# pema99/rust-path-tracer

Hardware: AMD Instinct MI355X
Metric: Mrays/s (higher is better)
Workload: dtype f32

## Files before the change

rust-path-tracer_amd/csrc/k_common.h:

```cpp
#ifndef RPT_K_COMMON_H
#define RPT_K_COMMON_H

#include <hip/hip_runtime.h>
#include <stdint.h>

#include "../../include/rpt/shared_structs.h"
#include "rpt_math.h"

#define RPT_WAVE 64
#define RPT_BLOCK 256
#define RPT_MAX_SAMPLES_IN_FLIGHT 256u

struct F3 { float x, y, z; };
RPT_HD F3 f3(float x, float y, float z) { return F3{x, y, z}; }
RPT_HD F3 f3s(float s) { return F3{s, s, s}; }
RPT_HD F3 operator+(F3 a, F3 b) { return F3{a.x + b.x, a.y + b.y, a.z + b.z}; }
RPT_HD F3 operator-(F3 a, F3 b) { return F3{a.x - b.x, a.y - b.y, a.z - b.z}; }
RPT_HD F3 operator*(F3 a, F3 b) { return F3{a.x * b.x, a.y * b.y, a.z * b.z}; }
RPT_HD F3 operator*(F3 a, float s) { return F3{a.x * s, a.y * s, a.z * s}; }
RPT_HD F3 operator*(float s, F3 a) { return F3{s * a.x, s * a.y, s * a.z}; }
RPT_HD F3 operator/(F3 a, float s) { return F3{a.x / s, a.y / s, a.z / s}; }
RPT_HD F3 operator-(F3 a) { return F3{-a.x, -a.y, -a.z}; }
RPT_HD float dot3(F3 a, F3 b) { return (a.x * b.x) + (a.y * b.y) + (a.z * b.z); }
__device__ __forceinline__ F3 cross3(F3 a, F3 b) {
// ... 69 lines not shown
    uint32_t n_slots;
    uint32_t n_pixels;
    uint32_t group_shift;
    uint32_t q_shift;
};
RPT_HD size_t rpt_pixel_index(uint32_t pxy, uint32_t width) { return (size_t)(pxy >> 16) * width + (pxy & 0xffffu); }

#define FLAG_BOUNCE(f) ((f) & 0xffu)
#define FLAG_LOBE_SPEC(f) (((f) >> 8) & 1u)
#define FLAG_DIM(f) (((f) >> 16) & 0x3fu)
#define MAKE_FLAGS(bounce, spec, dim) (((bounce) & 0xffu) | ((uint32_t)(spec) << 8) | ((uint32_t)(dim) << 16))
#define HIT_MISS 0xffffffffu
#define HIT_PENDING 0xfffffffeu
#define HIT_PARKED 0xfffffffdu
#define HIT_DONE 0xfffffffcu
#define HIT_IDLE 0xfffffffbu

#define Q_LINE 32
enum {  Q_ALIVE0 = 2 * Q_LINE, Q_ALIVE1 = 3 * Q_LINE, Q_REGEN0 = 4 * Q_LINE,
       Q_REGEN1 = 5 * Q_LINE, Q_DRAINED = 6 * Q_LINE, Q_POOL0 = 7 * Q_LINE, Q_POOL1 = 8 * Q_LINE, Q_SPOOL = 9 * Q_LINE, Q_COUNT = 12 * Q_LINE };
#define RPT_Q_SHARDS 16
#define RPT_Q_SHARD_STRIDE 1088
#define RPT_Q_SLACK (RPT_Q_SHARDS * (2048u + 256u))
__host__ __device__ __forceinline__ uint32_t q_position(uint32_t shard, uint32_t e) { return ((((e >> 8) * RPT_Q_SHARDS) | shard) << 8) | (e & 255u); }
__device__ __forceinline__ bool q_filled(const uint32_t *cnt, uint32_t p) {
    return ((((p >> 8) / RPT_Q_SHARDS) << 8) | (p & 255u)) < cnt[((p >> 8) % RPT_Q_SHARDS) * RPT_Q_SHARD_STRIDE];
}
__device__ __forceinline__ void q_extent(const uint32_t *cnt, uint32_t &positions, uint32_t &total) {
    uint32_t most = 0u, sum = 0u;
    for (uint32_t s = 0; s < RPT_Q_SHARDS; ++s) {
        const uint32_t c = cnt[s * RPT_Q_SHARD_STRIDE];
// ... 11 lines not shown
#define RPT_STAT_SHARDS 64
#define RPT_STAT_STRIDE 16

struct DevQueues {
    uint32_t *sky;
    float4 *sh_o;
    float4 *sh_d;
    float4 *sh_c;
    uint32_t *count;
    uint32_t *sky_cnt, *shadow_cnt;
    uint32_t sky_threshold;
    uint32_t known_length;
    uint32_t sky_at_end;
    uint32_t sky_wide_limit;
    uint32_t sky_shard_shift;
    unsigned long long *ray_shards;
    unsigned long long *host_ring;
    uint32_t ring_mask;
};

struct DevStats {
    unsigned long long extension_rays, shadow_rays, sky_evals, light_index_clamped, samples;
    unsigned long long undrained;
};

struct DevConfig {
    rpt_tracing_config c;
    float euler[9];
    float sky_rot[9];
    uint32_t nee_mode;
// ... 73 lines not shown
```

rust-path-tracer_amd/csrc/k_complete.h:

```cpp
#ifndef RPT_K_COMPLETE_H
#define RPT_K_COMPLETE_H

#include "k_path.h"
#include "k_moments.h"

#define RPT_COMPLETE_ROWS 32u
#define RPT_COMPLETE_PITCH 65u
__host__ __device__ __forceinline__ uint32_t complete_rows(uint32_t S) { return S < RPT_COMPLETE_ROWS ? S : RPT_COMPLETE_ROWS; }
__host__ __device__ __forceinline__ size_t complete_lds_bytes(uint32_t S, uint32_t q_shift) {
    return q_shift == 0u ? 0u : (size_t)complete_rows(S) * RPT_COMPLETE_PITCH * sizeof(float4) + (size_t)S * sizeof(unsigned long long);
}
template <uint32_t G>
__device__ __forceinline__ void complete_status_rows(const DevState &st, uint32_t base, uint32_t j0, uint32_t lane, unsigned long long *row_done, uint32_t my_group,
                                                     uint32_t my_shift, unsigned long long q_mask, uint32_t &n_done, uint32_t &n_busy, uint32_t &top) {
    const uint32_t gs = st.group_shift, qs = st.q_shift;
    uint32_t w[G];
#pragma unroll
    for (uint32_t i = 0u; i < G; ++i) w[i] = __float_as_uint(st.hit[base + ((j0 + i) << 6) + lane].y);
#pragma unroll
    for (uint32_t i = 0u; i < G; ++i) {
        const uint32_t row = j0 + i;
        const bool done = w[i] == HIT_DONE;
        const unsigned long long md = rpt_ballot(done), mb = rpt_ballot(!done && w[i] != HIT_IDLE);
        if (qs != 0u && lane == 0u) row_done[row] = md;
        if ((row >> (gs - qs)) == my_group) {
            const uint32_t bits = (uint32_t)((md >> my_shift) & q_mask);
            n_done += (uint32_t)__popc(bits);
            n_busy += (uint32_t)__popc((uint32_t)((mb >> my_shift) & q_mask));
            if (bits != 0u) top = ((row & ((1u << (gs - qs)) - 1u)) << qs) + 32u - (uint32_t)__clz((int)bits);
        }
    }
}
__device__ __forceinline__ uint32_t complete_block_slot(const DevState &st, uint32_t base, uint32_t kb, uint32_t t, uint32_t rows, uint32_t rows_log, uint32_t lane) {
    const uint32_t gs = st.group_shift, qs = st.q_shift;
    const uint32_t g = t >> (rows_log - qs), jl = (kb >> qs) + (t & ((rows >> qs) - 1u));
    return base + (((g << (gs - qs)) | jl) << 6) + lane;
}
template <uint32_t G>
__device__ __forceinline__ bool complete_stage_rows(const DevState &st, uint32_t base, uint32_t kb, uint32_t t0, uint32_t rows, uint32_t rows_log, uint32_t lane, float4 *tile,
                                                    const unsigned long long *row_done, unsigned long long ok_mask) {
    float rx[G], ry[G], rz[G], rw[G];
    uint32_t slot_of[G];
    bool restart = false;
#pragma unroll
    for (uint32_t i = 0u; i < G; ++i) {
        slot_of[i] = complete_block_slot(st, base, kb, t0 + i, rows, rows_log, lane);
        const float4 r = st.rad[slot_of[i]];
        rx[i] = r.x; ry[i] = r.y; rz[i] = r.z; rw[i] = r.w;
    }
#pragma unroll
    for (uint32_t i = 0u; i < G; ++i) {
        const uint32_t slot = slot_of[i], p = slot_pix(st, slot) & 63u, k = slot_k(st, slot);
        tile[(k - kb) * RPT_COMPLETE_PITCH + p] = make_float4(rx[i], ry[i], rz[i], rw[i]);
        const bool mine = ((row_done[(slot - base) >> 6] >> lane) & 1ull) != 0ull && ((ok_mask >> p) & 1ull) != 0ull;
        const uint32_t todo = __float_as_uint(rw[i]);
        if (mine && todo == 0u) st.hit[slot] = make_float2(0.0f, __uint_as_float(HIT_IDLE));
        restart = restart || rpt_ballot(mine && todo != 0u) != 0ull;
    }
    return restart;
}
__device__ __forceinline__ bool complete_restart_rows(const DevState &st, const DevConfig &cfg, uint32_t base, uint32_t kb, uint32_t rows, uint32_t rows_log, uint32_t lane,
                                                      const float4 *tile, const unsigned long long *row_done, unsigned long long ok_mask, uint32_t new_n, uint32_t rng_offset) {
// ... 31 lines not shown
```

rust-path-tracer_amd/csrc/k_complete_body.h:

```cpp
template <uint32_t G>
__device__ __forceinline__ bool RPT_COMPLETE_DIRECT_ROWS(const DevState &st, uint32_t base, uint32_t k0, uint32_t lane, bool ok, uint32_t n_done, float4 &acc RPT_MOM(, float4 &mom)) {
    float rx[G], ry[G], rz[G], rw[G];
    bool restart = false;
#pragma unroll
    for (uint32_t i = 0u; i < G; ++i) {
        const float4 r = st.rad[base + ((k0 + i) << 6) + lane];
        rx[i] = r.x; ry[i] = r.y; rz[i] = r.z; rw[i] = r.w;
    }
#pragma unroll
    for (uint32_t i = 0u; i < G; ++i) {
        const bool mine = ok && k0 + i < n_done;
        if (mine) { acc.x += rx[i]; acc.y += ry[i]; acc.z += rz[i]; acc.w += 1.0f; }
        RPT_MOM(if (mine) mo_add(mom, rx[i], ry[i], rz[i]);)
        const uint32_t todo = __float_as_uint(rw[i]);
        if (mine && todo == 0u) st.hit[base + ((k0 + i) << 6) + lane] = make_float2(0.0f, __uint_as_float(HIT_IDLE));
        restart = restart || rpt_ballot(mine && todo != 0u) != 0ull;
    }
    return restart;
}
__global__ __launch_bounds__(RPT_WAVE) void RPT_COMPLETE_KERNEL(DevState st, DevQueues q, DevConfig cfg, uint32_t iteration, uint32_t final_pass,
                                                                DevStats *stats RPT_MOM(, float4 *moments )) {
    if (!final_pass && q.count[Q_DRAINED] != 0u) return;
    extern __shared__ float4 complete_lds[];
    const uint32_t gs = st.group_shift, qs = st.q_shift, S = 1u << gs, rows = complete_rows(S);
    float4 *tile = complete_lds;
    unsigned long long *row_done = reinterpret_cast<unsigned long long *>(complete_lds + rows * RPT_COMPLETE_PITCH);
    const uint32_t lane = threadIdx.x, base = blockIdx.x << (6u + gs), pix = (blockIdx.x << 6) | lane;
    const bool in_image = pix < st.n_pixels;
    const uint32_t my_group = lane >> (6u - qs), my_shift = (lane & ((64u >> qs) - 1u)) << qs;
    const unsigned long long q_mask = (1ull << (1u << qs)) - 1ull;
    uint32_t n_done = 0u, n_busy = 0u, top = 0u;
    bool nothing_to_do = false;
    if (S >= 8u) {
        for (uint32_t j0 = 0u; j0 < S && !nothing_to_do; j0 += 8u) {
            complete_status_rows<8>(st, base, j0, lane, row_done, my_group, my_shift, q_mask, n_done, n_busy, top);
            nothing_to_do = !final_pass && rpt_ballot(in_image && n_busy == 0u) == 0ull;
        }
    } else if (S == 4u) complete_status_rows<4>(st, base, 0u, lane, row_done, my_group, my_shift, q_mask, n_done, n_busy, top);
    else complete_status_rows<2>(st, base, 0u, lane, row_done, my_group, my_shift, q_mask, n_done, n_busy, top);
    if (nothing_to_do) return;
    const bool ok = in_image && n_busy == 0u && n_done != 0u && top == n_done;
    if (final_pass && in_image && (n_busy != 0u || top != n_done)) {
        atomicAdd(&stats->undrained, (unsigned long long)(n_done + n_busy));
    }
    const unsigned long long ok_mask = rpt_ballot(ok);
    bool started = false;
    if (ok_mask != 0ull) {
        float4 acc = make_float4(0.0f, 0.0f, 0.0f, 0.0f);
        RPT_MOM(float4 mom = make_float4(0.0f, 0.0f, 0.0f, 0.0f);)
        uint2 rs = make_uint2(0u, 0u);
        if (ok) { acc = st.accum[pix]; rs = st.rng[pix]; }
        RPT_MOM(if (ok) mom = moments[pix];)
        const uint32_t new_n = rs.x + n_done;
        uint32_t most = ok ? n_done : 0u;
        for (uint32_t o = 32u; o != 0u; o >>= 1) { const uint32_t other = (uint32_t)__shfl_xor((int)most, (int)o, RPT_WAVE); most = other > most ? other : most; }
        const uint32_t rows_log = 31u - (uint32_t)__clz((int)rows);
        __syncthreads();
        if (qs == 0u) {
            const uint32_t G = S >= 8u ? 8u : S;
            for (uint32_t k0 = 0u; k0 < most; k0 += G) {
                bool restart;
                if (G == 8u) restart = RPT_COMPLETE_DIRECT_ROWS<8>(st, base, k0, lane, ok, n_done, acc RPT_MOM(, mom));
                else if (G == 4u) restart = RPT_COMPLETE_DIRECT_ROWS<4>(st, base, k0, lane, ok, n_done, acc RPT_MOM(, mom));
                else restart = RPT_COMPLETE_DIRECT_ROWS<2>(st, base, k0, lane, ok, n_done, acc RPT_MOM(, mom));
                if (restart) {
#pragma unroll 1
                    for (uint32_t k = k0; k < k0 + G; ++k) {
                        const uint32_t slot = base + (k << 6) + lane, todo = __float_as_uint(st.rad[slot].w);
                        if (ok && k < n_done && todo != 0u) {
                            start_path(st, cfg, slot, new_n + k, rs.y, todo - 1u);
                            started = true;
                        }
                    }
                }
            }
        } else
        for (uint32_t kb = 0u; kb < most; kb += rows) {
            bool restart = false;
            if (rows >= 8u) {
                for (uint32_t t0 = 0u; t0 < rows; t0 += 8u) restart |= complete_stage_rows<8>(st, base, kb, t0, rows, rows_log, lane, tile, row_done, ok_mask);
            } else if (rows == 4u) restart = complete_stage_rows<4>(st, base, kb, 0u, rows, rows_log, lane, tile, row_done, ok_mask);
            else restart = complete_stage_rows<2>(st, base, kb, 0u, rows, rows_log, lane, tile, row_done, ok_mask);
            __syncthreads();
            const uint32_t here = most - kb < rows ? most - kb : rows;
            for (uint32_t kl = 0u; kl < here; ++kl) {
                const float4 r = tile[kl * RPT_COMPLETE_PITCH + lane];
                if (ok && kb + kl < n_done) { acc.x += r.x; acc.y += r.y; acc.z += r.z; acc.w += 1.0f; }
                RPT_MOM(if (ok && kb + kl < n_done) mo_add(mom, r.x, r.y, r.z);)
            }
            if (restart) started |= complete_restart_rows(st, cfg, base, kb, rows, rows_log, lane, tile, row_done, ok_mask, new_n, rs.y);
            __syncthreads();
        }
        if (ok) {
            st.accum[pix] = acc;
            rs.x = new_n;
            st.rng[pix] = rs;
            RPT_MOM(moments[pix] = mom;)
// ... 6 lines not shown
```

rust-path-tracer_amd/csrc/k_path.h:

```cpp
#ifndef RPT_K_PATH_H
#define RPT_K_PATH_H

#include "k_common.h"

__device__ __forceinline__ F3 mat3_mul(const float *m, F3 v) {
    F3 r = f3(m[0], m[1], m[2]) * v.x;
    r = r + (f3(m[3], m[4], m[5]) * v.y);
    r = r + (f3(m[6], m[7], m[8]) * v.z);
    return r;
}

__device__ __forceinline__ void camera_ray(const DevConfig &cfg, uint32_t px, uint32_t py, uint32_t key, F3 &ro, F3 &rd) {
    Rng rng{key, 0u};
    float j1 = rng.next(), j2 = rng.next();
    float sx = (float)px + j1, sy = (float)py + j2;
    float ux = (sx / (float)cfg.c.width) * 2.0f - 1.0f;
    float uy = (1.0f - sy / (float)cfg.c.height) * 2.0f - 1.0f;
    uy *= (float)cfg.c.height / (float)cfg.c.width;
    ro = f3(cfg.c.cam_position[0], cfg.c.cam_position[1], cfg.c.cam_position[2]);
    rd = mat3_mul(cfg.euler, norm3(f3(ux, uy, 1.0f)));
}

__device__ __forceinline__ void start_path(const DevState &st, const DevConfig &cfg, uint32_t slot, uint32_t n, uint32_t offset,
                                           uint32_t todo_after) {
// ... 39 lines not shown
__device__ __forceinline__ void finish_in_side_stage(const DevState &st, const DevConfig &cfg, uint32_t slot, F3 radiance, uint32_t todo) {
    if (st.group_shift == 0u) {
        float4 acc = st.accum[slot];
        acc.x += radiance.x; acc.y += radiance.y; acc.z += radiance.z; acc.w += 1.0f;
        st.accum[slot] = acc;
        uint2 rs = st.rng[slot];
        rs.x += 1u;
        st.rng[slot] = rs;
        if (todo == 0u) st.hit[slot] = make_float2(0.0f, __uint_as_float(HIT_IDLE));
        else start_path(st, cfg, slot, rs.x, rs.y, todo - 1u);
    } else {
        st.rad[slot] = make_float4(radiance.x, radiance.y, radiance.z, __uint_as_float(todo));
        st.hit[slot] = make_float2(0.0f, __uint_as_float(HIT_DONE));
    }
}

#endif
```

rust-path-tracer_amd/csrc/k_shade.h:

```cpp
#ifndef RPT_K_SHADE_H
#define RPT_K_SHADE_H

#include "k_common.h"
#include "k_path.h"

#define RPT_PI_F 3.14159265358979323846f
#define RPT_EPS 0.001f

__device__ __forceinline__ uint32_t image_wrap(int32_t c, uint32_t extent, bool pow2) {
    if (pow2) return (uint32_t)c & (extent - 1u);
    const uint32_t u = (uint32_t)c;
    if (u < extent) return u;
    if (u == extent) return 0u;
    return (uint32_t)((uint64_t)(int64_t)c % (uint64_t)extent);
}
__device__ __forceinline__ float4 lerp4(float4 a, float4 b, float s) {
    return make_float4(a.x + ((b.x - a.x) * s), a.y + ((b.y - a.y) * s), a.z + ((b.z - a.z) * s), a.w + ((b.w - a.w) * s));
}
__device__ __forceinline__ float4 texel_of_u8(uint32_t t) {
    return make_float4(rptm::unorm8((float)(t & 0xffu)), rptm::unorm8((float)((t >> 8) & 0xffu)), rptm::unorm8((float)((t >> 16) & 0xffu)), 1.0f);
}
__device__ __forceinline__ void u8_row_pair(const uint32_t *texels, uint32_t row , uint32_t x0, uint32_t x1, uint32_t width, uint32_t &t0, uint32_t &t1) {
    const bool edge = x0 + 1u >= width;
    uint2 pair;
// ... 107 lines not shown
        m.metallic = make_float4(b.w, 0, 0, 0);
        m.normals = make_float4(0, 0, 0, 0);
        m.has = make_uint4(0u, 0u, 0u, 0u);
    }
    return m;
}


template <int NEE, bool TEXTURED, bool COMPACT>
__device__ __forceinline__ void shade_slot(const DevScene &sc, const DevState &st, const DevQueues &q, const DevConfig &cfg, DevStats *stats,
                                           uint32_t slot, float2 hw, bool active, bool &to_sky, bool &emit_shadow, float4 &sh_o, float4 &sh_d,
                                           float4 &sh_c, bool first ,
                                           uint32_t n_samples, bool &elided ,
                                           bool last_iteration ) {
    const uint32_t hit_tri = __float_as_uint(hw.y);
    if (NEE == RPT_NEE_NONE && last_iteration && active && hit_tri != HIT_MISS) {
        const uint32_t tri_index = hit_tri & 0x7fffffffu;
        const uint32_t m = __float_as_uint(sc.tri_shade[4u * tri_index + 2u].w);
        const float4 e4 = TEXTURED ? sc.materials[6u * m] : sc.mat_lite[2u * m];
        const bool emits = (e4.x != 0.0f || e4.y != 0.0f || e4.z != 0.0f) && (hit_tri >> 31) == 0u;
        if (emits || st.group_shift == 0u) {
            const float4 r4 = st.rad[slot];
            F3 radiance = f3(r4.x, r4.y, r4.z);
            if (emits) {
                const float4 tf = st.thr[slot];
                radiance = radiance + mask_nan3(f3(tf.x, tf.y, tf.z) * f3(e4.x, e4.y, e4.z));
            }
            finish_in_side_stage(st, cfg, slot, radiance, __float_as_uint(r4.w));
        } else {
            st.hit[slot] = make_float2(0.0f, __uint_as_float(HIT_DONE));
        }
        return;
    }
    if (active) {
        const float4 ra = st.ray_a[slot];
        const float2 rb = st.ray_b[slot];
        const F3 ro = f3(ra.x, ra.y, ra.z), rd = f3(ra.w, rb.x, rb.y);
        const float hit_t = hw.x;
        if (hit_tri == HIT_MISS) {
            to_sky = true;
            st.hit[slot] = make_float2(0.0f, __uint_as_float(HIT_PARKED));
            if (first) {
                st.thr[slot] = make_float4(1.0f, 1.0f, 1.0f, __uint_as_float(RPT_FRESH_FLAGS));
                st.rad[slot] = make_float4(0.0f, 0.0f, 0.0f, __uint_as_float(first_path_todo(st, slot, n_samples)));
            }
        } else {
            const float4 tf = first ? make_float4(1.0f, 1.0f, 1.0f, __uint_as_float(RPT_FRESH_FLAGS)) : st.thr[slot];
            F3 throughput = f3(tf.x, tf.y, tf.z);
            F3 radiance = f3s(0.0f);
            uint32_t todo = 0u;
            bool rad_loaded = false;
            auto load_rad = [&]() {
                if (!rad_loaded) {
                    if (first) {
                        todo = first_path_todo(st, slot, n_samples);
                    } else {
                        const float4 r4 = st.rad[slot];
                        radiance = f3(r4.x, r4.y, r4.z);
                        todo = __float_as_uint(r4.w);
                    }
                    rad_loaded = true;
                }
            };
            const uint32_t flags = __float_as_uint(tf.w);
            const uint32_t bounce = FLAG_BOUNCE(flags);
            const bool last_spec = FLAG_LOBE_SPEC(flags) != 0u;
            constexpr bool nee = NEE != RPT_NEE_NONE;
            const bool backface = (hit_tri >> 31) != 0u;
            const uint32_t tri_index = hit_tri & 0x7fffffffu;
            const float4 *ts = sc.tri_shade + 4u * tri_index;
            const float4 s0 = ts[0], s1 = ts[1], s2 = ts[2];
            const Mat mat = load_material<TEXTURED>(sc, __float_as_uint(s2.w));
            const F3 hit = ro + rd * hit_t;

            bool done = false;
            const F3 emissive = xyz4(mat.emissive);
            if (emissive.x != 0.0f || emissive.y != 0.0f || emissive.z != 0.0f) {
                if (backface) {
                    done = true;
                } else if (!nee || bounce == 0u || last_spec) {
                    load_rad();
                    radiance = radiance + mask_nan3(throughput * emissive);
                    done = true;
                } else if (NEE == RPT_NEE_MIS) {
                    const float4 ma = st.mis_a[slot], mb = st.mis_b[slot];
                    const uint32_t code = __float_as_uint(ma.x);
                    F3 contribution = f3s(0.0f);
                    if (code != 0xffffffffu) {
                        const rpt_light_pick_entry e = sc.light_pick[code >> 1];
                        const bool side_b = (code & 1u) != 0u;
                        const uint32_t light_tri = side_b ? e.triangle_index_b : e.triangle_index_a;
                        if (tri_index == light_tri) {
                            const float4 *lr = sc.light_rec + 8u * (code >> 1) + (side_b ? 4u : 0u);
                            const float light_area = side_b ? e.triangle_area_b : e.triangle_area_a;
                            const float light_pick_pdf = side_b ? e.triangle_pick_pdf_b : e.triangle_pick_pdf_a;
                            F3 light_normal = f3(lr[0].w, lr[1].w, lr[2].w);
                            float cos_theta = dot3(light_normal, -rd);
// ... 191 lines not shown
                    throughput = throughput * (spectrum / pdf);
                    new_d = sdir;
                    new_o = hit + sdir * RPT_EPS;
                    if (bounce > cfg.c.min_bounces) {
                        float prob = rptm::fmaxr(throughput.x, rptm::fmaxr(throughput.y, throughput.z));
                        if (rng.next() > prob) {
                            done = true;
                        } else {
                            throughput = throughput * (1.0f / prob);
                        }
                    }
                    new_flags = MAKE_FLAGS(bounce + 1u, spec ? 1u : 0u, rng.dim);
                }
            }

            if (done && !emit_shadow) {
                load_rad();
                finish_in_side_stage(st, cfg, slot, radiance, todo);
            } else {
                if (first) {
                    load_rad();
                    st.rad[slot] = make_float4(radiance.x, radiance.y, radiance.z, __uint_as_float(todo));
                }
                if (!done) {
                    st.thr[slot] = make_float4(throughput.x, throughput.y, throughput.z, __uint_as_float(new_flags));
                    st.ray_a[slot] = make_float4(new_o.x, new_o.y, new_o.z, new_d.x);
                    st.ray_b[slot] = make_float2(new_d.y, new_d.z);
                    st.hit[slot] = make_float2(0.0f, __uint_as_float(HIT_PENDING));
                    sh_d.w = __uint_as_float(slot);
                } else {
                    st.hit[slot] = make_float2(0.0f, __uint_as_float(HIT_PARKED));
                    sh_d.w = __uint_as_float(slot | 0x80000000u);
                }
            }
        }
// ... 136 lines not shown
```

rust-path-tracer_amd/csrc/k_sky_generate.h:

```cpp
#ifndef RPT_K_SKY_GENERATE_H
#define RPT_K_SKY_GENERATE_H

#include "k_shade.h"

#define SKY_EARTH_RADIUS 6360e3f
#define SKY_ATMOSPHERE_RADIUS 6380e3f
#define SKY_H_RAY 8e3f
#define SKY_H_MIE 12e2f

__device__ __forceinline__ float sky_escape(F3 p, F3 d, float r) {
    F3 v = p - f3(0.0f, -SKY_EARTH_RADIUS, 0.0f);
    float b = dot3(v, d);
    float det = b * b - dot3(v, v) + r * r;
    if (det < 0.0f) return -1.0f;
    det = rptm::sqrtr(det);
    float t1 = -b - det;
    float t2 = -b + det;
    return t1 >= 0.0f ? t1 : t2;
}
__device__ __forceinline__ float2 sky_densities(F3 p) {
    float h = rptm::fmaxr(len3(p - f3(0.0f, -SKY_EARTH_RADIUS, 0.0f)) - SKY_EARTH_RADIUS, 0.0f);
    return make_float2(rptm::exp_sky(rptm::div_const_nontiny(-h, SKY_H_RAY, 1.0f / SKY_H_RAY)),
                       rptm::exp_sky(rptm::div_const_nontiny(-h, SKY_H_MIE, 1.0f / SKY_H_MIE)));
}
// ... 75 lines not shown
    uint32_t i = blockIdx.x * RPT_BLOCK + threadIdx.x;
    uint32_t positions, n;
    q_extent(q.sky_cnt, positions, n);
    const uint32_t alive = q.count[Q_ALIVE0 + (iteration & 1u) * Q_LINE];
    const uint32_t drained = q.count[Q_DRAINED];
    if (i == 0u) {
        uint32_t busy = drained ? 0u : (alive | q.count[Q_REGEN0 + (iteration & 1u) * Q_LINE] | (n != 0u ? 1u : 0u));
        if (busy == 0u && drained == 0u) q.count[Q_DRAINED] = 1u;
        __hip_atomic_store(&q.host_ring[iteration & q.ring_mask], ((unsigned long long)(iteration + 1u) << 32) | busy,
                           __ATOMIC_RELEASE, __HIP_MEMORY_SCOPE_SYSTEM);
    }
    if (drained != 0u) return;
    if (q.sky_at_end == 0u && n < q.sky_threshold && alive != 0u) return;
    if (i == 0u && n) atomicAdd(&stats->sky_evals, (unsigned long long)n);
    const uint32_t stride = STRIDED ? gridDim.x * RPT_BLOCK : 0u;
    if (cfg.c.has_skybox == 0u && positions <= q.sky_wide_limit) {
        for (uint32_t m = i >> 4; m < positions; m += stride >> 4) {
            if (!q_filled(q.sky_cnt, m)) {
                if (!STRIDED) break;
                continue;
            }
            const uint32_t slot = q.sky[m];
            const uint32_t lane = __lane_id(), g0 = lane & ~15u, j = lane & 15u;
            float4 ra = st.ray_a[slot];
            float2 rb = st.ray_b[slot];
            F3 ro = f3(ra.x, ra.y, ra.z), rd = f3(ra.w, rb.x, rb.y);
            F3 sky = sky_scatter_wide(cfg.c.sun_direction, ro, rd, j, g0);
            if (j == 0u) {
                const float4 tf = st.thr[slot], r4 = st.rad[slot];
                F3 throughput = f3(tf.x, tf.y, tf.z), radiance = f3(r4.x, r4.y, r4.z);
                radiance = radiance + throughput * sky;
                finish_in_side_stage(st, cfg, slot, radiance, __float_as_uint(r4.w));
            }
            if (!STRIDED) break;
        }
        return;
    }
    for (; i < positions; i += stride) {
        if (!q_filled(q.sky_cnt, i)) {
            if (!STRIDED) break;
            continue;
        }
        uint32_t slot = q.sky[i];
        float4 ra = st.ray_a[slot];
        float2 rb = st.ray_b[slot];
        F3 ro = f3(ra.x, ra.y, ra.z), rd = f3(ra.w, rb.x, rb.y);
        const float4 tf = st.thr[slot], r4 = st.rad[slot];
        F3 throughput = f3(tf.x, tf.y, tf.z), radiance = f3(r4.x, r4.y, r4.z);
        if (cfg.c.has_skybox == 0u) {
            radiance = radiance + throughput * sky_scatter(cfg.c.sun_direction, ro, rd);
        } else {
            F3 rotated = mat3_mul(cfg.sky_rot, rd);
            float u = 0.5f + rptm::atan2r(rotated.z, rotated.x) / (2.0f * RPT_PI_F);
            float v = 1.0f - (0.5f + rptm::asinr(rotated.y) / RPT_PI_F);
            float intensity = cfg.c.sun_direction[3] * (1.0f / 15.0f);
            float4 s = sample_by_lod<false>(sc.skybox, u, v);
            radiance = radiance + throughput * f3(s.x, s.y, s.z) * intensity;
        }
        finish_in_side_stage(st, cfg, slot, radiance, __float_as_uint(r4.w));
        if (!STRIDED) break;
    }
}
// ... 43 lines not shown
```

rust-path-tracer_amd/csrc/k_traverse.h:

```cpp
#ifndef RPT_K_TRAVERSE_H
#define RPT_K_TRAVERSE_H

#include "k_common.h"
#include "k_path.h"
#include "rpt_fastdiv.h"

template <bool SMALL> struct StackElem { typedef uint32_t type; };
template <> struct StackElem<true> { typedef uint16_t type; };
template <typename T> __device__ __forceinline__ void stack_put(T *s, int sp, uint32_t v) { s[sp * RPT_WAVE] = (T)v; }
template <typename T> __device__ __forceinline__ uint32_t stack_get(T *s, int sp) { return (uint32_t)s[sp * RPT_WAVE]; }
struct Stack24 {
    uint16_t *lo;
    uint8_t *hi;
};
__device__ __forceinline__ void stack_put(Stack24 s, int sp, uint32_t v) {
    s.lo[sp * RPT_WAVE] = (uint16_t)v;
    s.hi[sp * RPT_WAVE] = (uint8_t)(v >> 16);
}
__device__ __forceinline__ uint32_t stack_get(Stack24 s, int sp) { return (uint32_t)s.lo[sp * RPT_WAVE] | ((uint32_t)s.hi[sp * RPT_WAVE] << 16); }
template <int K> struct StackBits {
    uint16_t *lo;
    uint32_t hi[K];
};
template <int K> __device__ __forceinline__ void stack_put(StackBits<K> &s, int sp, uint32_t v) {
// ... 672 lines not shown
        __syncthreads();
    }
    const SceneViewLds view = FIRST ? SceneViewLds{lds_scene, sc.lds_pairs, sc.n_triangles, sc.lds_root} : stage_scene_lds<THREADS>(sc, lds_scene);
    const float4 *img_lane = view.img;
    uint32_t stop_first = 0u;
    float order_bias = 0.0f;
    uint16_t *stack = &lds_stack[wave][0][lane];
    F3 ro = f3(0, 0, 0), rd = f3(1, 1, 1), ird = f3(1, 1, 1);
    LdsWalk w;
    lds_walk_begin(view, w);
    w.cur = LDS_DESC_DEAD;
    uint32_t slot = 0u;
    bool have = false;
    bool pool_open = true;
    uint32_t traced = 0u;
    const bool done_here = LAST && st.group_shift != 0u;
    auto last_finish = [&](uint32_t s, const HitRecord &r, uint32_t stopped) -> bool {
        if (!done_here) {
            st.hit[s] = make_float2(r.t, __uint_as_float(r.tri));
            return false;
        }
        if (r.tri == HIT_MISS) return true;
        if (stopped == 0u) {
            const uint32_t m = __float_as_uint(sc.tri_shade[4u * (r.tri & 0x7fffffffu) + 2u].w);
            const float4 e4 = sc.textured != 0u ? sc.materials[6u * m] : sc.mat_lite[2u * m];
            if ((e4.x != 0.0f || e4.y != 0.0f || e4.z != 0.0f) && (r.tri >> 31) == 0u) {
                float4 r4 = st.rad[s];
                const float4 tf = st.thr[s];
                const F3 radiance = f3(r4.x, r4.y, r4.z) + mask_nan3(f3(tf.x, tf.y, tf.z) * f3(e4.x, e4.y, e4.z));
                r4.x = radiance.x; r4.y = radiance.y; r4.z = radiance.z;
                st.rad[s] = r4;
            }
        }
        st.hit[s] = make_float2(0.0f, __uint_as_float(HIT_DONE));
        return false;
    };
    auto last_park = [&](bool park, uint32_t s) {
        const uint32_t shard = (s >> q.sky_shard_shift) % RPT_Q_SHARDS;
        unsigned long long todo_m = rpt_ballot(park);
        while (todo_m != 0ull) {
            const uint32_t leader = (uint32_t)__ffsll((long long)todo_m) - 1u;
            const uint32_t sh = (uint32_t)__builtin_amdgcn_readlane((int)shard, (int)leader);
            const bool mine = park && shard == sh;
            const unsigned long long same = rpt_ballot(mine);
            uint32_t e = 0u;
            if (lane == leader) e = atomicAdd(&q.sky_cnt[sh * RPT_Q_SHARD_STRIDE], (uint32_t)__popcll(same));
            e = (uint32_t)__builtin_amdgcn_readlane((int)e, (int)leader);
            if (mine) {
                e += __builtin_amdgcn_mbcnt_hi((uint32_t)(same >> 32), __builtin_amdgcn_mbcnt_lo((uint32_t)same, 0u));
// ... 231 lines not shown
```

rust-path-tracer_amd/csrc/rpt_hip.hip:

```cpp
#include <algorithm>
#include <cstdlib>
#include <cstring>

#include "rpt_ctx.h"

#include "k_shade.h"
#include "k_complete.h"
#include "k_sky_generate.h"
#include "k_image_order.h"

rpt_knobs rpt_read_knobs() {
    rpt_knobs k;
    auto num = [](const char *name, int lo, int hi, int otherwise) { const char *e = getenv(name); if (!e || !e[0]) return otherwise; const int v = atoi(e); return v < lo ? lo : (v > hi ? hi : v); };
    auto word = [](const char *name) { const char *e = getenv(name); return std::string(e ? e : ""); };
    k.stage_timing = num("RPT_STAGE_TIMING", 0, 2, 0);
    k.upload_timing = num("RPT_UPLOAD_TIMING", 0, 1, 0) == 1;
    k.slot_q_shift = num("RPT_SLOT_Q_SHIFT", 0, 5, -1);
    const std::string so = word("RPT_SHADOW_ORDER"), lo = word("RPT_LAST_ORDER");
    k.shadow_order = so == "near" ? 0 : (so == "fixed" ? 1 : -1);
    k.last_order = lo == "off" ? 4 : (lo == "near" ? 0 : (lo == "opaque" ? 1 : (lo == "small" ? 2 : (lo == "ratio" ? 3 : -1))));
    k.shade_compact = num("RPT_SHADE_COMPACT", 0, 1, -1);
    k.sky_strided = num("RPT_SKY_STRIDED", 0, 1 << 20, -1);
    k.stack_bits = num("RPT_STACK_BITS", 16, 32, 16);
    k.coop_leaves = num("RPT_COOP_LEAVES", 0, 1, -1);
// ... 75 lines not shown
    HIP_TRY(c, hipMemsetAsync(c->ray_shards.p, 0, RPT_STAT_SHARDS * RPT_STAT_STRIDE * sizeof(unsigned long long), c->stream));
    HIP_TRY(c, c->q_count.alloc(Q_WORDS));
    HIP_TRY(c, c->pixel_xy.alloc(np));
    if (np) HIP_TRY(c, hipMemcpy(c->pixel_xy.p, c->pixel_xy_host.data(), np * sizeof(uint32_t), hipMemcpyHostToDevice));
    HIP_TRY(c, hipMemsetAsync(c->q_count.p, 0, Q_WORDS * sizeof(uint32_t), c->stream));
    DevState &s = c->state;
    s = DevState{};
    s.rng = c->rng.p; s.accum = c->accum.p; s.pixel_xy = c->pixel_xy.p; s.n_slots = c->n_slots;
    s.n_pixels = (uint32_t)np; s.group_shift = c->group_shift; s.q_shift = 0;
    DevQueues &q = c->queues;
    q = DevQueues{};
    q.ray_shards = c->ray_shards.p; q.count = c->q_count.p;
    q.sky_cnt = c->q_count.p + Q_COUNT; q.shadow_cnt = q.sky_cnt + RPT_Q_SHARDS * RPT_Q_SHARD_STRIDE;
    q.host_ring = c->host_ring_dev; q.ring_mask = RING - 1;
    q.sky_wide_limit = (uint32_t)std::min<size_t>(c->n_slots / 16, c->sky_wide_cfg);
    q.sky_threshold = 1u; q.sky_at_end = 0u; q.known_length = 0u;
    c->has_state = true;
    return RPT_OK;
}

static uint32_t padded_pixels(uint32_t n_pixels) { return (n_pixels + 63u) & ~63u; }

static void launch_complete(rpt_ctx *c, uint32_t iteration, uint32_t final_pass) {
    if (c->moments_on) {
        k_complete_moments<<<padded_pixels(c->n_pixels) / RPT_WAVE, RPT_WAVE, complete_lds_bytes(1u << c->group_shift, c->state.q_shift), c->stream>>>(c->state, c->queues, c->cfg, iteration,
                                                                                                                                 final_pass, c->dev_stats.p, c->moments.p);
        return;
    }
    k_complete<<<padded_pixels(c->n_pixels) / RPT_WAVE, RPT_WAVE, complete_lds_bytes(1u << c->group_shift, c->state.q_shift), c->stream>>>(c->state, c->queues, c->cfg, iteration, final_pass,
                                                                                                                     c->dev_stats.p);
}
// ... 358 lines not shown
    const uint64_t known_iterations =
        (n_samples <= (1u << c->group_shift) && c->queues.sky_threshold <= 1u) ? (uint64_t)c->cfg.c.max_bounces : 0u;
    HIP_TRY(c, hipSetDevice(c->device));
    const auto t0 = std::chrono::steady_clock::now();
    hipStream_t s = c->stream;
    StageTimer &t = c->timing;
    const uint32_t blocks = rpt_blocks(c->n_slots);
    const bool async = allow_async && known_iterations != 0;
    if (!async && c->async_pending) {
        RPT_TRY(rpt_wait(c));
    }
    if (!async) for (int k = 0; k < RING; ++k) __atomic_store_n(&c->host_ring.p[k], 0ull, __ATOMIC_RELAXED);
    c->call_samples = n_samples;
    c->queues.sky_at_end = known_iterations != 0 ? 1u : 0u;
    c->queues.known_length = known_iterations != 0 ? 1u : 0u;
    c->queues.sky_shard_shift = c->shade_compact ? 11u : 8u;
    static_assert(RPT_BLOCK == 1 << 8 && RPT_BLOCK * RPT_SHADE_ROUNDS == 1 << 11, "sky_shard_shift: slots per workgroup of k_shade");
    t.mark(s, StageTimer::NONE, StageTimer::AT_1);
    c->first_walk_starts = rpt_first_walk_starts_paths(c);
    k_generate_first<<<c->first_walk_starts ? 1u : blocks, RPT_BLOCK, 0, s>>>(c->state, c->queues, c->cfg, n_samples, c->dev_stats.p, c->first_walk_starts ? 1u : 0u);
    c->stats.kernel_launches[RPT_STAGE_GENERATE] += 1;
    t.mark(s, RPT_STAGE_GENERATE, StageTimer::AT_1);

    const uint64_t planned = known_iterations - (async && known_iterations > 1 && c->test_short_batch ? 1u : 0u);
    const bool complete_each = known_iterations == 0 && c->group_shift != 0;
    const uint64_t lag = c->n_slots >= (512u << 10) ? 2 : (c->n_slots >= (128u << 10) ? 3 : LAG);
    const uint64_t it_limit = (uint64_t)n_samples * (uint64_t)(c->cfg.c.max_bounces + 2u) * 16u + 4096u;
    uint64_t it = 0, shade_launches = 0;
    bool drained = c->cfg.c.max_bounces == 0u;
    while (!drained) {
// ... 126 lines not shown
```

rust-path-tracer_amd/csrc/rpt_traverse.hip:

```cpp
#include <hip/hip_runtime.h>

#include <type_traits>

#include "rpt_ctx.h"
#include "k_traverse.h"

namespace {

constexpr int GLOBAL_THREADS = 64;
constexpr int LDS_THREADS = 1024;


template <int STACK>
static int gstream_stack_width(const rpt_ctx *c) {
    if (STACK == 16) return 16;
    const int bits = c->knobs.stack_bits;
    const int w = (c->scene.n_nodes < 65536u && bits <= 16) ? 16 : (c->scene.n_nodes < (1u << 21) && bits <= 21) ? 21 : (c->scene.n_nodes < (1u << 24) && bits <= 24) ? 24 : 32;
    return STACK == 24 && w > 24 ? 24 : w;
}
template <int STACK, typename F>
static void with_stack_width(int width, F &&launch) {
    if constexpr (STACK == 16) launch(std::integral_constant<int, 16>{});
    else if (width == 16) launch(std::integral_constant<int, 16>{});
    else if (width == 21) launch(std::integral_constant<int, 21>{});
// ... 26 lines not shown
}

template <int STACK>
bool launch_nearest(rpt_ctx *c, uint32_t iteration, bool last_without_nee = false ,
                    bool camera_rays = false ,
                    bool start_paths = false ) {
    hipStream_t s = c->stream;
    DevStats *stats = c->dev_stats.p;
    if (STACK == 16 && c->scene.lds_scene) {
        const size_t lds_bytes = (size_t)c->scene.lds_vecs * sizeof(float4);
        uint32_t grid;
        const uint32_t span = lds_stream_span(c, grid);
        const float *cam = c->cfg.c.cam_position;
        if (last_without_nee && c->scene.last_emit_n <= RPT_LAST_EMIT_MAX) {
            k_traverse_nearest_stream<16, LDS_THREADS, RPT_NEAREST_LAST><<<grid, LDS_THREADS, lds_bytes + (size_t)c->scene.last_flip_vecs * sizeof(float4), s>>>(c->scene, c->state, c->queues, iteration, span, 0.0f, 0.0f, 0.0f, c->cfg, 0u, stats);
            return c->state.group_shift != 0u;
        }
        if (camera_rays)
            k_traverse_nearest_stream<16, LDS_THREADS, RPT_NEAREST_FIRST><<<grid, LDS_THREADS, lds_bytes, s>>>(c->scene, c->state, c->queues, iteration, span, cam[0], cam[1], cam[2], c->cfg, start_paths ? c->call_samples : 0u, stats);
        else k_traverse_nearest_stream<16, LDS_THREADS><<<grid, LDS_THREADS, lds_bytes, s>>>(c->scene, c->state, c->queues, iteration, span, 0.0f, 0.0f, 0.0f, c->cfg, 0u, stats);
    } else if (c->scene.gpairs) {
        if (c->fat_leaves) launch_nearest_gstream<STACK, true>(c, iteration);
        else launch_nearest_gstream<STACK, false>(c, iteration);
    } else {
        const uint32_t nb = (c->n_slots + GLOBAL_THREADS - 1) / GLOBAL_THREADS;
        k_traverse_nearest<32, GLOBAL_THREADS><<<nb, GLOBAL_THREADS, 0, s>>>(c->scene, c->state, c->queues, iteration);
    }
    return false;
}

template <int STACK, bool COOP>
// ... 82 lines not shown
```

Baseline: 12860.

## Skip radiance buffer traffic for no-NEE known-length paths via implicit zero state

```diff
diff --git a/rust-path-tracer_amd/csrc/k_common.h b/rust-path-tracer_amd/csrc/k_common.h
--- a/rust-path-tracer_amd/csrc/k_common.h
+++ b/rust-path-tracer_amd/csrc/k_common.h
@@ -107,7 +107,8 @@
 #define HIT_PENDING 0xfffffffeu
 #define HIT_PARKED 0xfffffffdu
 #define HIT_DONE 0xfffffffcu
-#define HIT_IDLE 0xfffffffbu
+#define HIT_DONE_ZERO 0xfffffffbu
+#define HIT_IDLE 0xfffffffau
 
 #define Q_LINE 32
 enum {  Q_ALIVE0 = 2 * Q_LINE, Q_ALIVE1 = 3 * Q_LINE, Q_REGEN0 = 4 * Q_LINE,
@@ -149,6 +150,7 @@
     uint32_t sky_at_end;
     uint32_t sky_wide_limit;
     uint32_t sky_shard_shift;
+    uint32_t implicit_zero;
     unsigned long long *ray_shards;
     unsigned long long *host_ring;
     uint32_t ring_mask;
diff --git a/rust-path-tracer_amd/csrc/k_complete.h b/rust-path-tracer_amd/csrc/k_complete.h
--- a/rust-path-tracer_amd/csrc/k_complete.h
+++ b/rust-path-tracer_amd/csrc/k_complete.h
@@ -8,21 +8,22 @@
 #define RPT_COMPLETE_PITCH 65u
 __host__ __device__ __forceinline__ uint32_t complete_rows(uint32_t S) { return S < RPT_COMPLETE_ROWS ? S : RPT_COMPLETE_ROWS; }
 __host__ __device__ __forceinline__ size_t complete_lds_bytes(uint32_t S, uint32_t q_shift) {
-    return q_shift == 0u ? 0u : (size_t)complete_rows(S) * RPT_COMPLETE_PITCH * sizeof(float4) + (size_t)S * sizeof(unsigned long long);
+    return (size_t)((S + 7u) / 8u) * RPT_WAVE + (q_shift == 0u ? 0u : (size_t)complete_rows(S) * RPT_COMPLETE_PITCH * sizeof(float4) + (size_t)S * sizeof(unsigned long long));
 }
 template <uint32_t G>
-__device__ __forceinline__ void complete_status_rows(const DevState &st, uint32_t base, uint32_t j0, uint32_t lane, unsigned long long *row_done, uint32_t my_group,
-                                                     uint32_t my_shift, unsigned long long q_mask, uint32_t &n_done, uint32_t &n_busy, uint32_t &top) {
+__device__ __forceinline__ void complete_status_rows(const DevState &st, uint32_t base, uint32_t j0, uint32_t lane, unsigned long long *row_done, uint8_t *own_rad, uint32_t my_group, uint32_t my_shift, unsigned long long q_mask, uint32_t &n_done, uint32_t &n_busy, uint32_t &top) {
     const uint32_t gs = st.group_shift, qs = st.q_shift;
     uint32_t w[G];
 #pragma unroll
     for (uint32_t i = 0u; i < G; ++i) w[i] = __float_as_uint(st.hit[base + ((j0 + i) << 6) + lane].y);
+    uint32_t own = 0u;
 #pragma unroll
     for (uint32_t i = 0u; i < G; ++i) {
         const uint32_t row = j0 + i;
-        const bool done = w[i] == HIT_DONE;
+        const bool has_rad = w[i] == HIT_DONE, done = has_rad || w[i] == HIT_DONE_ZERO;
         const unsigned long long md = rpt_ballot(done), mb = rpt_ballot(!done && w[i] != HIT_IDLE);
         if (qs != 0u && lane == 0u) row_done[row] = md;
+        own |= (has_rad ? 1u : 0u) << i;
         if ((row >> (gs - qs)) == my_group) {
             const uint32_t bits = (uint32_t)((md >> my_shift) & q_mask);
             n_done += (uint32_t)__popc(bits);
@@ -30,22 +31,33 @@
             if (bits != 0u) top = ((row & ((1u << (gs - qs)) - 1u)) << qs) + 32u - (uint32_t)__clz((int)bits);
         }
     }
+    own_rad[(j0 >> 3) * RPT_WAVE + lane] = (uint8_t)own;
 }
 __device__ __forceinline__ uint32_t complete_block_slot(const DevState &st, uint32_t base, uint32_t kb, uint32_t t, uint32_t rows, uint32_t rows_log, uint32_t lane) {
     const uint32_t gs = st.group_shift, qs = st.q_shift;
     const uint32_t g = t >> (rows_log - qs), jl = (kb >> qs) + (t & ((rows >> qs) - 1u));
     return base + (((g << (gs - qs)) | jl) << 6) + lane;
 }
+__device__ __forceinline__ uint32_t complete_block_rad_bits(const DevState &st, uint32_t base, uint32_t kb, uint32_t rows, uint32_t rows_log, uint32_t lane, const uint8_t *own_rad) {
+    uint32_t bits = 0u;
+#pragma unroll 1
+    for (uint32_t t = 0u; t < rows; ++t) {
+        const uint32_t row = (complete_block_slot(st, base, kb, t, rows, rows_log, lane) - base) >> 6;
+        bits |= (((uint32_t)own_rad[(row >> 3) * RPT_WAVE + lane] >> (row & 7u)) & 1u) << t;
+    }
+    return bits;
+}
 template <uint32_t G>
 __device__ __forceinline__ bool complete_stage_rows(const DevState &st, uint32_t base, uint32_t kb, uint32_t t0, uint32_t rows, uint32_t rows_log, uint32_t lane, float4 *tile,
-                                                    const unsigned long long *row_done, unsigned long long ok_mask) {
+                                                    const unsigned long long *row_done, uint32_t rad_bits, unsigned long long ok_mask) {
     float rx[G], ry[G], rz[G], rw[G];
     uint32_t slot_of[G];
     bool restart = false;
 #pragma unroll
     for (uint32_t i = 0u; i < G; ++i) {
         slot_of[i] = complete_block_slot(st, base, kb, t0 + i, rows, rows_log, lane);
-        const float4 r = st.rad[slot_of[i]];
+        float4 r = make_float4(0.0f, 0.0f, 0.0f, __uint_as_float(0u));
+        if (((rad_bits >> (t0 + i)) & 1u) != 0u) r = st.rad[slot_of[i]];
         rx[i] = r.x; ry[i] = r.y; rz[i] = r.z; rw[i] = r.w;
     }
 #pragma unroll
diff --git a/rust-path-tracer_amd/csrc/k_complete_body.h b/rust-path-tracer_amd/csrc/k_complete_body.h
--- a/rust-path-tracer_amd/csrc/k_complete_body.h
+++ b/rust-path-tracer_amd/csrc/k_complete_body.h
@@ -1,10 +1,12 @@
 template <uint32_t G>
-__device__ __forceinline__ bool RPT_COMPLETE_DIRECT_ROWS(const DevState &st, uint32_t base, uint32_t k0, uint32_t lane, bool ok, uint32_t n_done, float4 &acc RPT_MOM(, float4 &mom)) {
+__device__ __forceinline__ bool RPT_COMPLETE_DIRECT_ROWS(const DevState &st, uint32_t base, uint32_t k0, uint32_t lane, bool ok, uint32_t n_done, uint32_t rad_bits,
+                                                         float4 &acc RPT_MOM(, float4 &mom)) {
     float rx[G], ry[G], rz[G], rw[G];
     bool restart = false;
 #pragma unroll
     for (uint32_t i = 0u; i < G; ++i) {
-        const float4 r = st.rad[base + ((k0 + i) << 6) + lane];
+        float4 r = make_float4(0.0f, 0.0f, 0.0f, __uint_as_float(0u));
+        if (ok && k0 + i < n_done && ((rad_bits >> i) & 1u) != 0u) r = st.rad[base + ((k0 + i) << 6) + lane];
         rx[i] = r.x; ry[i] = r.y; rz[i] = r.z; rw[i] = r.w;
     }
 #pragma unroll
@@ -25,6 +27,7 @@
     const uint32_t gs = st.group_shift, qs = st.q_shift, S = 1u << gs, rows = complete_rows(S);
     float4 *tile = complete_lds;
     unsigned long long *row_done = reinterpret_cast<unsigned long long *>(complete_lds + rows * RPT_COMPLETE_PITCH);
+    uint8_t *own_rad = qs == 0u ? reinterpret_cast<uint8_t *>(complete_lds) : reinterpret_cast<uint8_t *>(row_done + S);
     const uint32_t lane = threadIdx.x, base = blockIdx.x << (6u + gs), pix = (blockIdx.x << 6) | lane;
     const bool in_image = pix < st.n_pixels;
     const uint32_t my_group = lane >> (6u - qs), my_shift = (lane & ((64u >> qs) - 1u)) << qs;
@@ -33,11 +36,11 @@
     bool nothing_to_do = false;
     if (S >= 8u) {
         for (uint32_t j0 = 0u; j0 < S && !nothing_to_do; j0 += 8u) {
-            complete_status_rows<8>(st, base, j0, lane, row_done, my_group, my_shift, q_mask, n_done, n_busy, top);
+            complete_status_rows<8>(st, base, j0, lane, row_done, own_rad, my_group, my_shift, q_mask, n_done, n_busy, top);
             nothing_to_do = !final_pass && rpt_ballot(in_image && n_busy == 0u) == 0ull;
         }
-    } else if (S == 4u) complete_status_rows<4>(st, base, 0u, lane, row_done, my_group, my_shift, q_mask, n_done, n_busy, top);
-    else complete_status_rows<2>(st, base, 0u, lane, row_done, my_group, my_shift, q_mask, n_done, n_busy, top);
+    } else if (S == 4u) complete_status_rows<4>(st, base, 0u, lane, row_done, own_rad, my_group, my_shift, q_mask, n_done, n_busy, top);
+    else complete_status_rows<2>(st, base, 0u, lane, row_done, own_rad, my_group, my_shift, q_mask, n_done, n_busy, top);
     if (nothing_to_do) return;
     const bool ok = in_image && n_busy == 0u && n_done != 0u && top == n_done;
     if (final_pass && in_image && (n_busy != 0u || top != n_done)) {
@@ -60,14 +63,17 @@
             const uint32_t G = S >= 8u ? 8u : S;
             for (uint32_t k0 = 0u; k0 < most; k0 += G) {
                 bool restart;
-                if (G == 8u) restart = RPT_COMPLETE_DIRECT_ROWS<8>(st, base, k0, lane, ok, n_done, acc RPT_MOM(, mom));
-                else if (G == 4u) restart = RPT_COMPLETE_DIRECT_ROWS<4>(st, base, k0, lane, ok, n_done, acc RPT_MOM(, mom));
-                else restart = RPT_COMPLETE_DIRECT_ROWS<2>(st, base, k0, lane, ok, n_done, acc RPT_MOM(, mom));
+                const uint32_t rad_bits = own_rad[(k0 >> 3) * RPT_WAVE + lane];
+                if (G == 8u) restart = RPT_COMPLETE_DIRECT_ROWS<8>(st, base, k0, lane, ok, n_done, rad_bits, acc RPT_MOM(, mom));
+                else if (G == 4u) restart = RPT_COMPLETE_DIRECT_ROWS<4>(st, base, k0, lane, ok, n_done, rad_bits, acc RPT_MOM(, mom));
+                else restart = RPT_COMPLETE_DIRECT_ROWS<2>(st, base, k0, lane, ok, n_done, rad_bits, acc RPT_MOM(, mom));
                 if (restart) {
 #pragma unroll 1
                     for (uint32_t k = k0; k < k0 + G; ++k) {
-                        const uint32_t slot = base + (k << 6) + lane, todo = __float_as_uint(st.rad[slot].w);
-                        if (ok && k < n_done && todo != 0u) {
+                        const uint32_t slot = base + (k << 6) + lane;
+                        const bool has_rad = ok && k < n_done && ((rad_bits >> (k - k0)) & 1u) != 0u;
+                        const uint32_t todo = has_rad ? __float_as_uint(st.rad[slot].w) : 0u;
+                        if (todo != 0u) {
                             start_path(st, cfg, slot, new_n + k, rs.y, todo - 1u);
                             started = true;
                         }
@@ -77,10 +83,11 @@
         } else
         for (uint32_t kb = 0u; kb < most; kb += rows) {
             bool restart = false;
+            const uint32_t rad_bits = complete_block_rad_bits(st, base, kb, rows, rows_log, lane, own_rad);
             if (rows >= 8u) {
-                for (uint32_t t0 = 0u; t0 < rows; t0 += 8u) restart |= complete_stage_rows<8>(st, base, kb, t0, rows, rows_log, lane, tile, row_done, ok_mask);
-            } else if (rows == 4u) restart = complete_stage_rows<4>(st, base, kb, 0u, rows, rows_log, lane, tile, row_done, ok_mask);
-            else restart = complete_stage_rows<2>(st, base, kb, 0u, rows, rows_log, lane, tile, row_done, ok_mask);
+                for (uint32_t t0 = 0u; t0 < rows; t0 += 8u) restart |= complete_stage_rows<8>(st, base, kb, t0, rows, rows_log, lane, tile, row_done, rad_bits, ok_mask);
+            } else if (rows == 4u) restart = complete_stage_rows<4>(st, base, kb, 0u, rows, rows_log, lane, tile, row_done, rad_bits, ok_mask);
+            else restart = complete_stage_rows<2>(st, base, kb, 0u, rows, rows_log, lane, tile, row_done, rad_bits, ok_mask);
             __syncthreads();
             const uint32_t here = most - kb < rows ? most - kb : rows;
             for (uint32_t kl = 0u; kl < here; ++kl) {
diff --git a/rust-path-tracer_amd/csrc/k_path.h b/rust-path-tracer_amd/csrc/k_path.h
--- a/rust-path-tracer_amd/csrc/k_path.h
+++ b/rust-path-tracer_amd/csrc/k_path.h
@@ -77,5 +77,10 @@
         st.hit[slot] = make_float2(0.0f, __uint_as_float(HIT_DONE));
     }
 }
+__device__ __forceinline__ void finish_from_zero(const DevState &st, uint32_t slot, F3 added) {
+    const F3 radiance = f3s(0.0f) + added;
+    st.rad[slot] = make_float4(radiance.x, radiance.y, radiance.z, __uint_as_float(0u));
+    st.hit[slot] = make_float2(0.0f, __uint_as_float(HIT_DONE));
+}
 
 #endif
diff --git a/rust-path-tracer_amd/csrc/k_shade.h b/rust-path-tracer_amd/csrc/k_shade.h
--- a/rust-path-tracer_amd/csrc/k_shade.h
+++ b/rust-path-tracer_amd/csrc/k_shade.h
@@ -145,12 +145,20 @@
                                            uint32_t n_samples, bool &elided ,
                                            bool last_iteration ) {
     const uint32_t hit_tri = __float_as_uint(hw.y);
+    const bool zero_rad = NEE == RPT_NEE_NONE && q.implicit_zero != 0u;
     if (NEE == RPT_NEE_NONE && last_iteration && active && hit_tri != HIT_MISS) {
         const uint32_t tri_index = hit_tri & 0x7fffffffu;
         const uint32_t m = __float_as_uint(sc.tri_shade[4u * tri_index + 2u].w);
         const float4 e4 = TEXTURED ? sc.materials[6u * m] : sc.mat_lite[2u * m];
         const bool emits = (e4.x != 0.0f || e4.y != 0.0f || e4.z != 0.0f) && (hit_tri >> 31) == 0u;
-        if (emits || st.group_shift == 0u) {
+        if (zero_rad) {
+            if (emits) {
+                const float4 tf = st.thr[slot];
+                finish_from_zero(st, slot, mask_nan3(f3(tf.x, tf.y, tf.z) * f3(e4.x, e4.y, e4.z)));
+            } else {
+                st.hit[slot] = make_float2(0.0f, __uint_as_float(HIT_DONE_ZERO));
+            }
+        } else if (emits || st.group_shift == 0u) {
             const float4 r4 = st.rad[slot];
             F3 radiance = f3(r4.x, r4.y, r4.z);
             if (emits) {
@@ -173,7 +181,7 @@
             st.hit[slot] = make_float2(0.0f, __uint_as_float(HIT_PARKED));
             if (first) {
                 st.thr[slot] = make_float4(1.0f, 1.0f, 1.0f, __uint_as_float(RPT_FRESH_FLAGS));
-                st.rad[slot] = make_float4(0.0f, 0.0f, 0.0f, __uint_as_float(first_path_todo(st, slot, n_samples)));
+                if (!zero_rad) st.rad[slot] = make_float4(0.0f, 0.0f, 0.0f, __uint_as_float(first_path_todo(st, slot, n_samples)));
             }
         } else {
             const float4 tf = first ? make_float4(1.0f, 1.0f, 1.0f, __uint_as_float(RPT_FRESH_FLAGS)) : st.thr[slot];
@@ -181,9 +189,11 @@
             F3 radiance = f3s(0.0f);
             uint32_t todo = 0u;
             bool rad_loaded = false;
+            bool added = false;
             auto load_rad = [&]() {
                 if (!rad_loaded) {
-                    if (first) {
+                    if (zero_rad) {
+                    } else if (first) {
                         todo = first_path_todo(st, slot, n_samples);
                     } else {
                         const float4 r4 = st.rad[slot];
@@ -212,6 +222,7 @@
                 } else if (!nee || bounce == 0u || last_spec) {
                     load_rad();
                     radiance = radiance + mask_nan3(throughput * emissive);
+                    added = true;
                     done = true;
                 } else if (NEE == RPT_NEE_MIS) {
                     const float4 ma = st.mis_a[slot], mb = st.mis_b[slot];
@@ -433,11 +444,13 @@
                 }
             }
 
-            if (done && !emit_shadow) {
+            if (zero_rad && done && !added) {
+                st.hit[slot] = make_float2(0.0f, __uint_as_float(HIT_DONE_ZERO));
+            } else if (done && !emit_shadow) {
                 load_rad();
                 finish_in_side_stage(st, cfg, slot, radiance, todo);
             } else {
-                if (first) {
+                if (first && !zero_rad) {
                     load_rad();
                     st.rad[slot] = make_float4(radiance.x, radiance.y, radiance.z, __uint_as_float(todo));
                 }
diff --git a/rust-path-tracer_amd/csrc/k_sky_generate.h b/rust-path-tracer_amd/csrc/k_sky_generate.h
--- a/rust-path-tracer_amd/csrc/k_sky_generate.h
+++ b/rust-path-tracer_amd/csrc/k_sky_generate.h
@@ -113,6 +113,7 @@
     if (q.sky_at_end == 0u && n < q.sky_threshold && alive != 0u) return;
     if (i == 0u && n) atomicAdd(&stats->sky_evals, (unsigned long long)n);
     const uint32_t stride = STRIDED ? gridDim.x * RPT_BLOCK : 0u;
+    const bool zero_rad = q.implicit_zero != 0u;
     if (cfg.c.has_skybox == 0u && positions <= q.sky_wide_limit) {
         for (uint32_t m = i >> 4; m < positions; m += stride >> 4) {
             if (!q_filled(q.sky_cnt, m)) {
@@ -126,7 +127,7 @@
             F3 ro = f3(ra.x, ra.y, ra.z), rd = f3(ra.w, rb.x, rb.y);
             F3 sky = sky_scatter_wide(cfg.c.sun_direction, ro, rd, j, g0);
             if (j == 0u) {
-                const float4 tf = st.thr[slot], r4 = st.rad[slot];
+                const float4 tf = st.thr[slot], r4 = zero_rad ? make_float4(0.0f, 0.0f, 0.0f, __uint_as_float(0u)) : st.rad[slot];
                 F3 throughput = f3(tf.x, tf.y, tf.z), radiance = f3(r4.x, r4.y, r4.z);
                 radiance = radiance + throughput * sky;
                 finish_in_side_stage(st, cfg, slot, radiance, __float_as_uint(r4.w));
@@ -144,7 +145,7 @@
         float4 ra = st.ray_a[slot];
         float2 rb = st.ray_b[slot];
         F3 ro = f3(ra.x, ra.y, ra.z), rd = f3(ra.w, rb.x, rb.y);
-        const float4 tf = st.thr[slot], r4 = st.rad[slot];
+        const float4 tf = st.thr[slot], r4 = zero_rad ? make_float4(0.0f, 0.0f, 0.0f, __uint_as_float(0u)) : st.rad[slot];
         F3 throughput = f3(tf.x, tf.y, tf.z), radiance = f3(r4.x, r4.y, r4.z);
         if (cfg.c.has_skybox == 0u) {
             radiance = radiance + throughput * sky_scatter(cfg.c.sun_direction, ro, rd);
diff --git a/rust-path-tracer_amd/csrc/k_traverse.h b/rust-path-tracer_amd/csrc/k_traverse.h
--- a/rust-path-tracer_amd/csrc/k_traverse.h
+++ b/rust-path-tracer_amd/csrc/k_traverse.h
@@ -710,7 +710,7 @@
     bool have = false;
     bool pool_open = true;
     uint32_t traced = 0u;
-    const bool done_here = LAST && st.group_shift != 0u;
+    const bool done_here = LAST && q.implicit_zero != 0u;
     auto last_finish = [&](uint32_t s, const HitRecord &r, uint32_t stopped) -> bool {
         if (!done_here) {
             st.hit[s] = make_float2(r.t, __uint_as_float(r.tri));
@@ -721,14 +721,12 @@
             const uint32_t m = __float_as_uint(sc.tri_shade[4u * (r.tri & 0x7fffffffu) + 2u].w);
             const float4 e4 = sc.textured != 0u ? sc.materials[6u * m] : sc.mat_lite[2u * m];
             if ((e4.x != 0.0f || e4.y != 0.0f || e4.z != 0.0f) && (r.tri >> 31) == 0u) {
-                float4 r4 = st.rad[s];
                 const float4 tf = st.thr[s];
-                const F3 radiance = f3(r4.x, r4.y, r4.z) + mask_nan3(f3(tf.x, tf.y, tf.z) * f3(e4.x, e4.y, e4.z));
-                r4.x = radiance.x; r4.y = radiance.y; r4.z = radiance.z;
-                st.rad[s] = r4;
-            }
-        }
-        st.hit[s] = make_float2(0.0f, __uint_as_float(HIT_DONE));
+                finish_from_zero(st, s, mask_nan3(f3(tf.x, tf.y, tf.z) * f3(e4.x, e4.y, e4.z)));
+                return false;
+            }
+        }
+        st.hit[s] = make_float2(0.0f, __uint_as_float(HIT_DONE_ZERO));
         return false;
     };
     auto last_park = [&](bool park, uint32_t s) {
diff --git a/rust-path-tracer_amd/csrc/rpt_hip.hip b/rust-path-tracer_amd/csrc/rpt_hip.hip
--- a/rust-path-tracer_amd/csrc/rpt_hip.hip
+++ b/rust-path-tracer_amd/csrc/rpt_hip.hip
@@ -113,7 +113,7 @@
     q.sky_cnt = c->q_count.p + Q_COUNT; q.shadow_cnt = q.sky_cnt + RPT_Q_SHARDS * RPT_Q_SHARD_STRIDE;
     q.host_ring = c->host_ring_dev; q.ring_mask = RING - 1;
     q.sky_wide_limit = (uint32_t)std::min<size_t>(c->n_slots / 16, c->sky_wide_cfg);
-    q.sky_threshold = 1u; q.sky_at_end = 0u; q.known_length = 0u;
+    q.sky_threshold = 1u; q.sky_at_end = 0u; q.known_length = 0u; q.implicit_zero = 0u;
     c->has_state = true;
     return RPT_OK;
 }
@@ -502,6 +502,7 @@
     c->call_samples = n_samples;
     c->queues.sky_at_end = known_iterations != 0 ? 1u : 0u;
     c->queues.known_length = known_iterations != 0 ? 1u : 0u;
+    c->queues.implicit_zero = (known_iterations != 0 && c->cfg.nee_mode == RPT_NEE_NONE && c->group_shift != 0u) ? 1u : 0u;
     c->queues.sky_shard_shift = c->shade_compact ? 11u : 8u;
     static_assert(RPT_BLOCK == 1 << 8 && RPT_BLOCK * RPT_SHADE_ROUNDS == 1 << 11, "sky_shard_shift: slots per workgroup of k_shade");
     t.mark(s, StageTimer::NONE, StageTimer::AT_1);
diff --git a/rust-path-tracer_amd/csrc/rpt_traverse.hip b/rust-path-tracer_amd/csrc/rpt_traverse.hip
--- a/rust-path-tracer_amd/csrc/rpt_traverse.hip
+++ b/rust-path-tracer_amd/csrc/rpt_traverse.hip
@@ -64,7 +64,7 @@
         const float *cam = c->cfg.c.cam_position;
         if (last_without_nee && c->scene.last_emit_n <= RPT_LAST_EMIT_MAX) {
             k_traverse_nearest_stream<16, LDS_THREADS, RPT_NEAREST_LAST><<<grid, LDS_THREADS, lds_bytes + (size_t)c->scene.last_flip_vecs * sizeof(float4), s>>>(c->scene, c->state, c->queues, iteration, span, 0.0f, 0.0f, 0.0f, c->cfg, 0u, stats);
-            return c->state.group_shift != 0u;
+            return c->queues.implicit_zero != 0u;
         }
         if (camera_rays)
             k_traverse_nearest_stream<16, LDS_THREADS, RPT_NEAREST_FIRST><<<grid, LDS_THREADS, lds_bytes, s>>>(c->scene, c->state, c->queues, iteration, span, cam[0], cam[1], cam[2], c->cfg, start_paths ? c->call_samples : 0u, stats);
```

Measured after the change: 13130 (median of 6 runs). 1.02x the previous value.
